# Tyler-Linchenwei/Graph-Distillation-for-Recommendation

Measured on AMD Instinct MI355X. Metric: distill wallclock (SpMM+k-means) & test-acc parity, ogbn-arxiv r=0.5% @1-8 GPU, higher is better.
Workload: dtype fp32

## Files before the change

### graph-distillation-for-recommendation_amd/csrc/gdd_propagate.hip

```cpp
#include <algorithm>
#include <cstdio>
#include <cstdlib>

#include "gdd_common.hpp"

namespace gdd {
namespace {

constexpr int kSeg = GDD_PROP_SEG;
constexpr int kUnroll = 8;

struct Item {
  int32_t row, begin, end, pslot;
};

template <int V>
struct VecT;
template <>
struct VecT<4> {
  using T = float4;
};
template <>
struct VecT<2> {
  using T = float2;
// ... 2 lines not shown
struct VecT<1> {
  using T = float;
};

template <int V>
__device__ __forceinline__ void vload(const float* p, float (&r)[V]) {
  if constexpr (V == 4) {
    float4 t = *reinterpret_cast<const float4*>(p);
    r[0] = t.x; r[1] = t.y; r[2] = t.z; r[3] = t.w;
  } else if constexpr (V == 2) {
    float2 t = *reinterpret_cast<const float2*>(p);
    r[0] = t.x; r[1] = t.y;
  } else {
    r[0] = *p;
  }
}
using f32x4 = __attribute__((ext_vector_type(4))) float;
using f32x2 = __attribute__((ext_vector_type(2))) float;
template <int V>
__device__ __forceinline__ void vload_nt(const float* p, float (&r)[V]) {
  if constexpr (V == 4) {
    f32x4 t = __builtin_nontemporal_load(reinterpret_cast<const f32x4*>(p));
    r[0] = t.x; r[1] = t.y; r[2] = t.z; r[3] = t.w;
  } else if constexpr (V == 2) {
    f32x2 t = __builtin_nontemporal_load(reinterpret_cast<const f32x2*>(p));
    r[0] = t.x; r[1] = t.y;
  } else {
    r[0] = __builtin_nontemporal_load(p);
  }
}
template <int V>
__device__ __forceinline__ void vstore_nt(float* p, const float (&r)[V]) {
  if constexpr (V == 4) {
    f32x4 t = {r[0], r[1], r[2], r[3]};
    __builtin_nontemporal_store(t, reinterpret_cast<f32x4*>(p));
  } else if constexpr (V == 2) {
    f32x2 t = {r[0], r[1]};
    __builtin_nontemporal_store(t, reinterpret_cast<f32x2*>(p));
  } else {
    __builtin_nontemporal_store(r[0], p);
  }
}
template <int V>
__device__ __forceinline__ void vstore(float* p, const float (&r)[V]) {
  if constexpr (V == 4) {
    *reinterpret_cast<float4*>(p) = make_float4(r[0], r[1], r[2], r[3]);
  } else if constexpr (V == 2) {
    *reinterpret_cast<float2*>(p) = make_float2(r[0], r[1]);
  } else {
    *p = r[0];
  }
}

__global__ void k_seg_counts(int64_t n, const int32_t* __restrict__ rowptr,
                             const int32_t* __restrict__ order, const int32_t* __restrict__ rowwise,
                             int32_t* nseg, int32_t* npart) {
  int64_t i = (int64_t)blockIdx.x * blockDim.x + threadIdx.x;
  if (i >= n) return;
  const int64_t r = (order && !(rowwise && *rowwise)) ? order[i] : i;
  int32_t len = rowptr[r + 1] - rowptr[r];
  int32_t s = len <= kSeg ? 1 : (len + kSeg - 1) / kSeg;
  nseg[i] = s;
  npart[i] = s > 1 ? s : 0;
}

__global__ void k_make_items(int64_t n, const int32_t* __restrict__ rowptr,
                             const int32_t* __restrict__ order, const int32_t* __restrict__ rowwise,
                             const int32_t* __restrict__ nseg, const int32_t* __restrict__ item_off,
                             const int32_t* __restrict__ part_off, Item* items,
                             int32_t* long_rows, int32_t* long_off, int32_t* counts) {
  int64_t i = (int64_t)blockIdx.x * blockDim.x + threadIdx.x;
  if (i >= n) return;
  const int32_t r = (order && !(rowwise && *rowwise)) ? order[i] : (int32_t)i;
  const int32_t b = rowptr[r], e = rowptr[r + 1], s = nseg[i], o = item_off[i];
  if (s == 1) {
    items[o] = Item{r, b, e, -1};
  } else {
    const int32_t po = part_off[i];
    for (int32_t k = 0; k < s; ++k) {
      int32_t lo = b + k * kSeg, hi = min(e, lo + kSeg);
      items[o + k] = Item{r, lo, hi, po + k};
    }
    int32_t q = atomicAdd(&counts[1], 1);
    long_rows[q] = r;
    long_off[q] = po;
  }
  if (i == n - 1) counts[0] = o + s;
}

constexpr int kProbeRows = 4096;
constexpr int kProbeCap = 64;
constexpr int kProbeWindow = 4096;
constexpr int64_t kProbeMinRows = 1000000;
__global__ __launch_bounds__(1024) void k_locality_probe(int64_t n, const int32_t* __restrict__ rowptr,
                                                         const int32_t* __restrict__ col,
                                                         int32_t* __restrict__ flag) {
  __shared__ unsigned long long tot[2];
  if (threadIdx.x < 2) tot[threadIdx.x] = 0;
  __syncthreads();
  unsigned near = 0, all = 0;
  const int64_t stride = n / kProbeRows;
  for (int q = threadIdx.x; q < kProbeRows; q += blockDim.x) {
    const int64_t r = q * stride;
    const int32_t b = rowptr[r], e = min(rowptr[r + 1], b + kProbeCap);
    for (int32_t p = b; p < e; ++p) {
      const int64_t dlt = (int64_t)col[p] - r;
      near += (dlt <= kProbeWindow && dlt >= -kProbeWindow) ? 1u : 0u;
    }
    all += (unsigned)(e - b);
  }
  atomicAdd(&tot[0], (unsigned long long)near);
  atomicAdd(&tot[1], (unsigned long long)all);
  __syncthreads();
  if (threadIdx.x == 0) flag[0] = (tot[1] > 0 && 2 * tot[0] >= tot[1]) ? 1 : 0;
}

constexpr int kLenKeyBits = 10;
constexpr int32_t kLenKeyMax = (1 << kLenKeyBits) - 1;
__global__ void k_len_keys(int64_t n, const int32_t* __restrict__ rowptr, int32_t* keys,
                           int32_t* rows) {
  int64_t i = (int64_t)blockIdx.x * blockDim.x + threadIdx.x;
  if (i >= n) return;
  keys[i] = kLenKeyMax - min(rowptr[i + 1] - rowptr[i], kLenKeyMax);
  rows[i] = (int32_t)i;
}

template <int V, int G, int S>
__global__ __launch_bounds__(256) void k_hop(const Item* __restrict__ items,
                                             const int32_t* __restrict__ counts,
                                             const int32_t* __restrict__ col,
                                             const float* __restrict__ val, float scale, int d,
                                             const float* __restrict__ x, float* __restrict__ y,
                                             float* __restrict__ acc_out, float acc_scale,
                                             const float* __restrict__ acc_init,
                                             const float* __restrict__ acc_prev,
                                             float* __restrict__ partials,
                                             const int32_t* __restrict__ ymap,
                                             const int32_t* __restrict__ pmap, int contig) {
  const int lane = threadIdx.x & (G - 1);
  int64_t ib;
  int chunk;
  if constexpr (S > 0) {
    const int xcd = blockIdx.x & 7;
    chunk = xcd % S;
    ib = contig ? (int64_t)xcd * (gridDim.x >> 3) + (blockIdx.x >> 3)
                : (int64_t)(blockIdx.x >> 3) * (8 / S) + xcd / S;
  } else {
    chunk = blockIdx.y;
    ib = blockIdx.x;
  }
  const int64_t g = (ib * blockDim.x + threadIdx.x) / G;
  if (g >= counts[0]) return;
  const Item it = items[g];
  const int f = (chunk * G + lane) * V;
  const bool fa = f < d;
  float acc[V];
#pragma unroll
  for (int v = 0; v < V; ++v) acc[v] = 0.f;

  for (int32_t c0 = it.begin; c0 < it.end; c0 += G) {
    const int32_t p = c0 + lane;
    const bool in = p < it.end;
    const int32_t cj = in ? __builtin_nontemporal_load(col + p) : 0;
    const float vj = in ? scale * __builtin_nontemporal_load(val + p) : 0.f;
    const int cnt = min(G, it.end - c0);
    for (int t = 0; t < cnt; t += kUnroll) {
      float xv[kUnroll][V];
      float vv[kUnroll];
#pragma unroll
      for (int u = 0; u < kUnroll; ++u) {
        const int src = t + u;
        const int32_t jj = __shfl(cj, src < G ? src : 0, G);
        vv[u] = __shfl(vj, src < G ? src : 0, G);
        if (src < cnt && fa) {
          vload<V>(x + (int64_t)jj * d + f, xv[u]);
        } else {
#pragma unroll
          for (int v = 0; v < V; ++v) xv[u][v] = 0.f;
        }
      }
#pragma unroll
      for (int u = 0; u < kUnroll; ++u) {
        if (t + u < cnt) {
#pragma unroll
          for (int v = 0; v < V; ++v) acc[v] = __builtin_fmaf(vv[u], xv[u][v], acc[v]);
        }
      }
    }
  }
  if (!fa) return;
  if (it.pslot < 0) {
    const int64_t o = (int64_t)it.row * d + f;
    const int64_t oy = ymap ? (int64_t)ymap[it.row] * d + f : o;
    vstore<V>(y + oy, acc);
    if (acc_out) {
      float t[V];
      if (acc_init) {
        vload_nt<V>(acc_init + o, t);
#pragma unroll
        for (int v = 0; v < V; ++v) t[v] = acc_scale * t[v];
      } else {
        vload_nt<V>(acc_out + o, t);
      }
      if (acc_prev) {
        float q[V];
        vload<V>(acc_prev + (pmap ? (int64_t)pmap[it.row] * d + f : o), q);
#pragma unroll
        for (int v = 0; v < V; ++v) t[v] = t[v] + acc_scale * q[v];
      }
#pragma unroll
      for (int v = 0; v < V; ++v) t[v] = t[v] + acc_scale * acc[v];
      vstore_nt<V>(acc_out + o, t);
    }
  } else {
    vstore<V>(partials + (int64_t)it.pslot * d + f, acc);
  }
}

constexpr int kFixupBlocks = 1024;
__global__ void k_fixup(const int32_t* __restrict__ counts, const int32_t* __restrict__ long_rows,
                        const int32_t* __restrict__ long_off, const int32_t* __restrict__ rowptr,
                        int d, const float* __restrict__ partials, float* __restrict__ y,
                        float* __restrict__ acc_out, float acc_scale,
                        const float* __restrict__ acc_init, const float* __restrict__ acc_prev,
                        const int32_t* __restrict__ ymap, const int32_t* __restrict__ pmap) {
  const int nl = counts[1];
  for (int r = blockIdx.x; r < nl; r += gridDim.x) {
    const int32_t row = long_rows[r], po = long_off[r];
    const int32_t len = rowptr[row + 1] - rowptr[row];
    const int32_t s = (len + kSeg - 1) / kSeg;
    for (int f = threadIdx.x; f < d; f += blockDim.x) {
      const float* pp = partials + (int64_t)po * d + f;
      float sum = pp[0];
      int32_t k = 1;
      for (; k + 8 <= s; k += 8) {
        float v[8];
#pragma unroll
        for (int u = 0; u < 8; ++u) v[u] = pp[(int64_t)(k + u) * d];
#pragma unroll
        for (int u = 0; u < 8; ++u) sum = sum + v[u];
      }
      for (; k < s; ++k) sum = sum + pp[(int64_t)k * d];
      const int64_t o = (int64_t)row * d + f;
      y[ymap ? (int64_t)ymap[row] * d + f : o] = sum;
      if (acc_out) {
        float t = acc_init ? acc_scale * acc_init[o] : acc_out[o];
        if (acc_prev) t = t + acc_scale * acc_prev[pmap ? (int64_t)pmap[row] * d + f : o];
        acc_out[o] = t + acc_scale * sum;
      }
    }
  }
}

__global__ void k_scale_copy(int64_t total, const float* __restrict__ x, float w,
                             float* __restrict__ target, float* __restrict__ copy) {
  int64_t i = (int64_t)blockIdx.x * blockDim.x + threadIdx.x;
  int64_t stride = (int64_t)gridDim.x * blockDim.x;
  for (; i < total; i += stride) {
    float v = x[i];
    target[i] = w * v;
    if (copy) copy[i] = v;
  }
}

struct Plan {
  Item* items;
  int32_t* counts;
  int32_t* long_rows;
  int32_t* long_off;
  float* partials;
  int64_t max_items;
  int64_t max_long;
  void* sort_ws;
  size_t sort_bytes;
};


inline int64_t max_items_for(int64_t n, int64_t nnz) { return n + nnz / kSeg + 1; }
inline int64_t max_parts_for(int64_t nnz) { return 2 * (nnz / kSeg) + 2; }

constexpr int kLenKeys = kLenKeyMax + 1;
size_t sched_ws_bytes(int64_t n) {
  return align256(sizeof(int32_t) * (kLenKeys + 1)) + align256(gdd_group_ws_bytes(n, kLenKeys));
}

size_t plan_ws_bytes(int64_t n, int64_t nnz, int d) {
  size_t b = 0;
  b += align256(sizeof(int32_t) * n) * 7;
  b += sched_ws_bytes(n);
  b += align256(sizeof(Item) * max_items_for(n, nnz));
  b += align256(sizeof(int32_t) * 4);
  b += align256(sizeof(int32_t) * (nnz / kSeg + 1)) * 2;
  b += align256(sizeof(float) * max_parts_for(nnz) * (size_t)d);
  b += scan_i32_ws_bytes(n) + 256;
  return b + 4096;
}

int carve_plan(int64_t n, int64_t nnz, int d, Carver& cv, Plan& pl, int32_t** tmp, void** scan_ws,
               size_t* scan_bytes) {
  for (int q = 0; q < 7; ++q) tmp[q] = cv.take<int32_t>(n);
  pl.max_items = max_items_for(n, nnz);
  pl.max_long = nnz / kSeg + 1;
  pl.items = cv.take<Item>(pl.max_items);
  pl.counts = cv.take<int32_t>(4);
  pl.long_rows = cv.take<int32_t>(pl.max_long);
  pl.long_off = cv.take<int32_t>(pl.max_long);
  pl.partials = cv.take<float>(max_parts_for(nnz) * (size_t)d);
  *scan_bytes = scan_i32_ws_bytes(n);
  *scan_ws = cv.take<char>(*scan_bytes);
  pl.sort_bytes = sched_ws_bytes(n);
  pl.sort_ws = cv.take<char>(pl.sort_bytes);
  if (!cv.ok()) return fail(GDD_E_WORKSPACE, "propagate: workspace too small");
  return GDD_OK;
}

int build_plan(int64_t n, int64_t nnz, int d, const int32_t* rowptr, const int32_t* col_for_probe,
               Carver& cv, Plan& pl, hipStream_t s, const int32_t* given_order = nullptr) {
  int32_t* tmp[7];
  void* scan_ws;
  size_t sb;
  int rc0 = carve_plan(n, nnz, d, cv, pl, tmp, &scan_ws, &sb);
  if (rc0) return rc0;
  int32_t *nseg = tmp[0], *npart = tmp[1], *item_off = tmp[2], *part_off = tmp[3];
  const unsigned gb = (unsigned)((n + 255) / 256);
  GDD_HIP(hipMemsetAsync(pl.counts, 0, sizeof(int32_t) * 4, s));
  const int32_t* order = given_order;
  const int32_t* rowwise = nullptr;
  if (!given_order && col_for_probe && n >= kProbeMinRows && !forced("hop_no_probe") &&
      !forced("hop_row_order")) {
    k_locality_probe<<<1, 1024, 0, s>>>(n, rowptr, col_for_probe, pl.counts + 2);
    GDD_LAUNCHED();
    rowwise = pl.counts + 2;
  }
  if (!given_order && !forced("hop_row_order")) {
    k_len_keys<<<gb, 256, 0, s>>>(n, rowptr, tmp[4], tmp[5]);
    GDD_LAUNCHED();
    Carver sc(pl.sort_ws, pl.sort_bytes);
    int32_t* key_off = sc.take<int32_t>(kLenKeys + 1);
    const size_t gws = gdd_group_ws_bytes(n, kLenKeys);
    void* gw = sc.take<char>(gws);
    if (!sc.ok()) return fail(GDD_E_WORKSPACE, "propagate: schedule workspace too small");
    int rc = gdd_group_by_label(n, tmp[4], kLenKeys, tmp[6], key_off, gw, gws,
                                reinterpret_cast<gdd_stream_t>(s));
    if (rc) return rc;
    order = tmp[6];
  }
  k_seg_counts<<<gb, 256, 0, s>>>(n, rowptr, order, rowwise, nseg, npart);
  GDD_LAUNCHED();
  int rc = exclusive_scan_i32(nseg, item_off, n, scan_ws, sb, s);
  if (rc) return rc;
  rc = exclusive_scan_i32(npart, part_off, n, scan_ws, sb, s);
  if (rc) return rc;
  k_make_items<<<gb, 256, 0, s>>>(n, rowptr, order, rowwise, nseg, item_off, part_off, pl.items,
                                  pl.long_rows, pl.long_off, pl.counts);
  GDD_LAUNCHED();
  return GDD_OK;
}

struct RowMaps {
  const int32_t* y;
  const int32_t* prev;
};

struct HopForm {
  int V, G, S;
};

HopForm hop_form(int d, int align) {
  if (d <= 0 || (align != 16 && align != 8 && align != 4)) return HopForm{0, 0, 0};
  const int V = (d % 4 == 0 && align == 16) ? 4 : (d % 2 == 0 && align >= 8) ? 2 : 1;
  const int lanes = (d + V - 1) / V;
  const int G = (lanes <= 16 || (V == 4 && lanes > 28 && lanes <= 32)) ? 16 : lanes <= 32 ? 32 : 64;
  const int chunks = (d + G * V - 1) / (G * V);
  const int S = (chunks == 8 || chunks == 4 || chunks == 2 || chunks == 1) ? chunks : 0;
  return HopForm{V, G, S};
}

template <int V, int G, int S>
void launch_hop(const Plan& pl, const int32_t* col, const float* val, float scale, int d,
                const float* x, float* y, float* acc, float acc_scale, const float* acc_init,
                const float* acc_prev, RowMaps rm, hipStream_t s) {
  constexpr int kGroups = 256 / G;
  const int64_t iblocks = (pl.max_items + kGroups - 1) / kGroups;
  if constexpr (S > 0) {
    const int64_t groups = (iblocks + (8 / S) - 1) / (8 / S);
    k_hop<V, G, S><<<(unsigned)(groups * 8), 256, 0, s>>>(pl.items, pl.counts, col, val, scale, d,
                                                          x, y, acc, acc_scale, acc_init, acc_prev,
                                                          pl.partials, rm.y, rm.prev,
                                                          S == 1 && forced("hop_xcd_contig") ? 1 : 0);
  } else {
    const int chunks = (d + G * V - 1) / (G * V);
    k_hop<V, G, 0><<<dim3((unsigned)iblocks, (unsigned)chunks), 256, 0, s>>>(
        pl.items, pl.counts, col, val, scale, d, x, y, acc, acc_scale, acc_init, acc_prev, pl.partials,
        rm.y, rm.prev, 0);
  }
}

template <int V, int G, class... A>
void launch_hop_vg(int S, const A&... a) {
  switch (S) {
    case 8: return launch_hop<V, G, 8>(a...);
    case 4: return launch_hop<V, G, 4>(a...);
    case 2: return launch_hop<V, G, 2>(a...);
    case 1: return launch_hop<V, G, 1>(a...);
    default: return launch_hop<V, G, 0>(a...);
  }
}

template <int V, class... A>
void launch_hop_v(HopForm f, const A&... a) {
  switch (f.G) {
    case 16: return launch_hop_vg<V, 16>(f.S, a...);
    case 32: return launch_hop_vg<V, 32>(f.S, a...);
    default: return launch_hop_vg<V, 64>(f.S, a...);
  }
}

int run_hop(const Plan& pl, const int32_t* rowptr, const int32_t* col, const float* val,
            float scale, int d, const float* x, float* y, float* acc, float acc_scale,
            hipStream_t s, const float* acc_init = nullptr, const float* acc_prev = nullptr,
            RowMaps rm = RowMaps{nullptr, nullptr}) {
  auto aligned = [](const void* p, int a) { return ((uintptr_t)p % a) == 0; };
  const bool a16 = aligned(x, 16) && aligned(y, 16) && (!acc || aligned(acc, 16)) &&
                   (!acc_init || aligned(acc_init, 16)) && (!acc_prev || aligned(acc_prev, 16)) &&
                   aligned(pl.partials, 16);
  const bool a8 = aligned(x, 8) && aligned(y, 8) && (!acc || aligned(acc, 8)) &&
                  (!acc_init || aligned(acc_init, 8)) && (!acc_prev || aligned(acc_prev, 8));
  const HopForm f = hop_form(d, a16 ? 16 : a8 ? 8 : 4);
  switch (f.V) {
    case 4:
      launch_hop_v<4>(f, pl, col, val, scale, d, x, y, acc, acc_scale, acc_init, acc_prev, rm, s);
      break;
    case 2:
      launch_hop_v<2>(f, pl, col, val, scale, d, x, y, acc, acc_scale, acc_init, acc_prev, rm, s);
      break;
    default:
      launch_hop_v<1>(f, pl, col, val, scale, d, x, y, acc, acc_scale, acc_init, acc_prev, rm, s);
      break;
  }
  GDD_LAUNCHED();
  const unsigned fixup_grid = (unsigned)std::min<int64_t>(pl.max_long, kFixupBlocks);
  k_fixup<<<fixup_grid, 256, 0, s>>>(pl.counts, pl.long_rows, pl.long_off, rowptr, d, pl.partials, y,
                                     acc, acc_scale, acc_init, acc_prev, rm.y, rm.prev);
  GDD_LAUNCHED();
  return GDD_OK;
}

int check_csr_args(int64_t n, int64_t nnz, const int32_t* rowptr, const int32_t* col,
                   const float* val, int d) {
  GDD_REQUIRE(n > 0 && n < INT32_MAX, "propagate: n=%lld out of range", (long long)n);
  GDD_REQUIRE(nnz >= 0 && nnz < INT32_MAX, "propagate: nnz=%lld out of range", (long long)nnz);
  GDD_REQUIRE(d > 0, "propagate: d=%d must be positive", d);
  GDD_REQUIRE(rowptr && (nnz == 0 || (col && val)), "propagate: null CSR pointer");
  return GDD_OK;
}

}
}

using namespace gdd;

extern "C" const char* gdd_hop_path(int d, int align) {
  static thread_local char name[32];
  const HopForm f = hop_form(d, align);
  if (f.V == 0) return "invalid";
  snprintf(name, sizeof name, "v%d/g%d/s%d", f.V, f.G, f.S);
  return name;
}

extern "C" size_t gdd_propagate_ws_bytes(int64_t n, int64_t nnz, int d) {
  return plan_ws_bytes(n, nnz, d);
}

extern "C" int gdd_spmm(int64_t n, int64_t nnz, const int32_t* rowptr, const int32_t* col,
                        const float* val, int d, float scale, const float* x, float* y, float* acc,
                        float acc_scale, void* ws, size_t ws_bytes, gdd_stream_t stream) {
  int rc = check_csr_args(n, nnz, rowptr, col, val, d);
  if (rc) return rc;
  GDD_REQUIRE(x && y && ws, "spmm: null pointer");
  hipStream_t s = to_hip(stream);
  Carver cv(ws, ws_bytes);
  Plan pl;
  rc = build_plan(n, nnz, d, rowptr, col, cv, pl, s);
  if (rc) return rc;
  return run_hop(pl, rowptr, col, val, scale, d, x, y, acc, acc_scale, s);
}

extern "C" int gdd_spmm_plan(int64_t n, int64_t nnz, const int32_t* rowptr, int d, void* ws,
                             size_t ws_bytes, gdd_stream_t stream) {
  GDD_REQUIRE(n > 0 && n < INT32_MAX && nnz >= 0 && nnz < INT32_MAX && d > 0 && rowptr && ws,
              "spmm_plan: bad arguments");
  Carver cv(ws, ws_bytes);
  Plan pl;
  return build_plan(n, nnz, d, rowptr, nullptr, cv, pl, to_hip(stream));
}

// ... 120 lines not shown
```

### graph-distillation-for-recommendation_amd/csrc/gdd_kmeanspp.hip

```cpp
#include <algorithm>
#include <climits>
#include <cmath>
#include <cstdlib>

#include <cstring>

#include "gdd_common.hpp"

namespace gdd {
GDD_STAMP_TABLE(kpp)
namespace {

constexpr int kMaxTrials = 16;
constexpr int kBlk = 4096;
constexpr int kThr = 1024;
constexpr int kWaves = kThr / 64;
constexpr int kPer = kBlk / kThr;
constexpr int kBlasThreads = 8;

struct KppState {
  float pot;
  int pad;
};

// ... 1285 lines not shown
      rl[t] = 0.0;
      exl[t] = 0.0;
      if (t < T) {
        float xs[kPer];
#pragma unroll
        for (int q = 0; q < kPer; ++q) xs[q] = s_d[t * kBlk + kPer * tid + q];
        double run = 0.0, r[kPer];
#pragma unroll
        for (int q = 0; q < kPer; ++q) {
          const int64_t e = j0 + kPer * tid + q;
          run = run + (e < n ? (double)(wv(a.w, e) * xs[q]) : 0.0);
          r[q] = run;
        }
        double inc = run;
#pragma unroll
        for (int o = 1; o < 64; o <<= 1) {
          const double y = __shfl_up(inc, o);
          if (lane >= o) inc = inc + y;
        }
        double ex = __shfl_up(inc, 1);
        if (lane == 0) ex = 0.0;
        if (lane == 63) s_wt[t][wave] = inc;
        exl[t] = ex;
#pragma unroll
        for (int q = 0; q < kPer; ++q)
          if (q == (int)(last % kPer)) rl[t] = r[q];
      }
    }
    __syncthreads();
    if (owner) {
#pragma unroll
      for (int t = 0; t < kSplitMaxT; ++t) {
        if (t < T) {
          double B = 0.0;
          for (int q = 0; q < wave; ++q) B = B + s_wt[t][q];
          a.fsum[cq][(int64_t)t * a.nblk + blk] = (B + exl[t]) + rl[t];
        }
      }
    }
  }
  GDD_STAMP_WHEN(g_stamps_kpp, (tid == 0 && c == 5 && (blk == 0 || blk == a.nblk - 1)), blk == 0 ? 34 : 44);
  const int64_t NB = min<int64_t>(kBlk, a.m1 - j0);
  if (NB > 0 && wave < T) {
    const float v = sgemv_block_wave(s_d + wave * kBlk, a.w ? a.w + j0 : nullptr, NB, wave, T);
    if (lane == 0) a.vblk[cq][(int64_t)wave * a.nblk + blk] = v;
  }
  GDD_STAMP_WHEN(g_stamps_kpp, (lane == 0 && wave == 0 && c == 5 && (blk == 0 || blk == a.nblk - 1)),
                 blk == 0 ? 35 : 45);
#ifdef GDD_STAMPS
  if (lane == 0 && c == 5) atomicMax(&g_stamps_kpp[46], (unsigned long long)__builtin_amdgcn_s_memrealtime());
#endif
}

__global__ __launch_bounds__(kThr) void k_kpp_final(KppArgs a, int c) {
  __shared__ float s_pot[kMaxTrials];
  const int q = c & 1;
  const int b = fold_round(a, q, s_pot);
  const int64_t src = a.cand[q][b];
  if (threadIdx.x == 0) a.indices[c] = src;
  for (int j = threadIdx.x; j < a.dim; j += kThr) a.centers[(int64_t)c * a.dim + j] = a.X[src * a.dim + j];
}

constexpr int kTg = 2;
constexpr int kPts = 64;

struct Kpp1Args {
  int64_t n, m1;
  int dim, T, k, pad;
  const float* X;
  const float* XT;
  const float* w;
  const double* xsq;
  const float* closest0;
  const KppState* st;
  const double* uniforms;
  float* dist[2];
  float* potv[2];
  int64_t* candw[2];
  int64_t* candself[2];
  int64_t* candr[2];
  double* candn[2];
  int* win;
  unsigned* counter;
  float* centers;
  int64_t* indices;
  SklPlan plan;
  float* dist2[2];
  float* potv2[2];
  int64_t* candw2[2];
  int64_t* candself2[2];
  int exact;
};

__device__ __forceinline__ int kpp1_argmin(const float* __restrict__ pot, int T) {
  int b = 0;
  for (int q = 1; q < T; ++q) {
    const float pb = pot[b], pt = pot[q];
    if (pb == pb && (pt < pb || pt != pt)) b = q;
  }
  return b;
}

template <bool SEQ>
__global__ __launch_bounds__(256) void k_kpp1_dist(Kpp1Args a, int c) {
  extern __shared__ double s_cr[];
  __shared__ int64_t s_cw[kMaxTrials * kMaxTrials];
// ... 1641 lines not shown
  const SklPlan p{n, B, T, dim, 0, 0};
  const int64_t ms[2] = {std::min(n, B), n > B ? n % B : 0};
  for (int64_t m : ms)
    if (m > 0 && !skl_chunk_seq(p, m)) return false;
  return true;
}

}
}

using namespace gdd;

extern "C" int gdd_skl_sqdist(int n_rows, const float* C, int64_t n, int dim, const float* X,
                              float* out, gdd_stream_t stream) {
  GDD_REQUIRE(n_rows >= 1 && n > 0 && dim > 0 && dim <= 4096, "skl_sqdist: invalid shape");
  GDD_REQUIRE(n <= (int64_t)INT_MAX * kThr, "skl_sqdist: n too large");
  GDD_REQUIRE(C && X && out, "skl_sqdist: null pointer");
  SklPlan p{n, skl_batch_size(n_rows, n, dim), n_rows, dim, 0, 0};
  p.all_seq = skl_all_seq(n, n_rows, dim, p.B) ? 1 : 0;
  const size_t lds = sizeof(double) * (size_t)dim;
  k_skl_sqdist<<<dim3((unsigned)((n + kThr - 1) / kThr), (unsigned)n_rows), kThr, lds,
                 to_hip(stream)>>>(p, C, X, out);
  GDD_LAUNCHED();
  return GDD_OK;
}

namespace {

enum KppPath {
  KPP_FIRST_ONLY,
  KPP_SINGLE_TABLE_PAIR,
  KPP_SINGLE_TABLE,
  KPP_SINGLE_FUSED,
  KPP_SINGLE_TWO_LAUNCH,
  KPP_SPLIT,
  KPP_BIG_PAIR,
  KPP_BIG,
  KPP_BLOCK_TABLE,
  KPP_BLOCK,
};

struct KppPlan {
  int64_t n, nblk;
  int dim, T, k;
  KppPath path;
  bool seq;
  int64_t B, B1;
  int exact;
  int overlap;
  int ept;
  size_t lds;
  size_t lds1;
  size_t lds_split;
  size_t lds_big;
  bool xt;
  bool xt_before_init;
  bool xt_after_first;
  bool Dbig;
  bool Dm;
  bool pairs;
};

constexpr int64_t kDmBigMax = 32768;
constexpr int64_t kBig1Default = 16384;
bool kpp_table_pays(int64_t n, int dim, int k) {
  return (double)(k - 1) * 2.5e7 >= (double)n * (double)n * (double)dim;
}

KppPlan kpp_plan(int64_t n, int dim_in, int n_trials, int k_in) {
  KppPlan p{};
  const int dim = p.dim = std::max(dim_in, 1);
  const int T = p.T = std::max(n_trials, 1);
  const int k = p.k = std::max(k_in, 1);
  p.n = n;
  p.nblk = (n + kBlk - 1) / kBlk;
  p.B = skl_batch_size(T, n, dim);
  p.B1 = skl_batch_size(1, n, dim);
  p.seq = skl_all_seq(n, T, dim, p.B);
  const char* ex = getenv("GDD_KPP_EXACT");
  p.exact = ex ? atoi(ex) : 1;
  p.overlap = forced("kpp_pair_serial") ? 0 : 1;
  p.ept = n <= (int64_t)kBigThr * 8 ? 8 : n <= (int64_t)kBigThr * 16 ? 16 : 32;
  p.lds = sizeof(double) * (size_t)dim + sizeof(float) * (kBlk + kChainPad);
  p.lds1 = sizeof(double) * (size_t)T * std::max(dim, 48);
  p.lds_split = sizeof(double) * (size_t)T * dim + sizeof(float) * (size_t)T * kBlk;
  p.lds_big = sizeof(float) * ((size_t)kBigThr * p.ept + kChainPad);

  const bool no_table = forced("kpp_no_table"), single_round = forced("kpp_single_round");
  const bool table_shape = dim <= kDmX && T >= 2 && k >= kDmMinK;
  p.xt = n <= kBlk || n * (int64_t)dim < INT_MAX;
  p.Dm = n <= kBlk && table_shape;
  p.Dbig = n > kBlk && n <= kDmBigMax && table_shape && !no_table &&
           (kpp_table_pays(n, dim, k) || forced("kpp_force_table")) && p.seq;
  p.pairs = p.Dm || (p.Dbig && T <= kPairMaxT && n <= (int64_t)kBigThr * 8);

  const bool single = p.nblk == 1 && T >= 2;
  p.xt_before_init = p.xt && n > kBlk;
  p.xt_after_first = single && p.seq && k > 1;
  const int64_t big1_max = std::min((int64_t)forced_value("kpp_big1_max", (double)kBig1Default), kBig1Max);
  const bool big1 = n <= big1_max && T >= 2 && !forced("kpp_no_big1");
  const bool split = p.seq && p.xt_before_init && T >= 2 && T <= kSplitMaxT && p.lds_split <= 150 * 1024 &&
                     p.nblk >= kSplitMinBlocks && !forced("kpp_no_split");
  if (k == 1) {
    p.path = KPP_FIRST_ONLY;
  } else if (single) {
    const int64_t fused_grid = (n + kFPts - 1) / kFPts * T;
    if (p.seq && p.Dm && !no_table)
      p.path = T <= kPairMaxT && !single_round ? KPP_SINGLE_TABLE_PAIR : KPP_SINGLE_TABLE;
    else if (dim <= kMaxDimF && fused_grid <= 256 && !forced("kpp_two_launch"))
      p.path = KPP_SINGLE_FUSED;
    else
      p.path = KPP_SINGLE_TWO_LAUNCH;
  } else if (split) {
    p.path = KPP_SPLIT;
  } else if (p.Dbig && p.xt_before_init) {
    p.path = !big1 ? KPP_BLOCK_TABLE : p.pairs && !single_round ? KPP_BIG_PAIR : KPP_BIG;
  } else {
    p.path = KPP_BLOCK;
  }
  return p;
}

const char* kpp_path_name(const KppPlan& p) {
  switch (p.path) {
    case KPP_FIRST_ONLY: return "first_only";
    case KPP_SINGLE_TABLE_PAIR: return "single_table_pair";
    case KPP_SINGLE_TABLE: return "single_table";
    case KPP_SINGLE_FUSED: return p.seq ? "single_fused/seq" : "single_fused/blas";
    case KPP_SINGLE_TWO_LAUNCH: return p.seq ? "single_two_launch/seq" : "single_two_launch/blas";
    case KPP_SPLIT: return "split";
    case KPP_BIG_PAIR: return "big_pair";
    case KPP_BIG: return "big";
    case KPP_BLOCK_TABLE: return "block_table";
    case KPP_BLOCK: return p.seq ? "block/seq" : "block/blas";
  }
  return "invalid";
}

struct KppBufs {
  KppState* st;
  double* xsq;
  float* closest0;
  double* fsum0;
  float* XT;
  float* Dbig;
  float* Dm;
};

void kpp_carve(const KppPlan& p, Carver& cv, KppBufs* bf, KppArgs* a, Kpp1Args* b1) {
  const size_t n = (size_t)p.n, nblk = (size_t)p.nblk, T = (size_t)p.T;
  bf->st = cv.take<KppState>(1);
  bf->xsq = cv.take<double>(n);
  bf->closest0 = cv.take<float>(n);
  bf->fsum0 = cv.take<double>(nblk);
  for (int q = 0; q < 2; ++q) a->dist[q] = cv.take<float>(n * T);
// ... 144 lines not shown
  struct {
    Kpp1Args b1;
    const float* Dm;
    int k, overlap;
  } key;
  std::memset(&key, 0, sizeof(key));
  key.b1 = b1;
  key.Dm = Dm;
  key.k = p.k;
  key.overlap = overlap;
  return replay_or_run("kpp_pair_chain", &key, sizeof(key), s, chain);
}

int kpp_single_table(const KppPlan& p, const KppBufs& bf, const Kpp1Args& b1, hipStream_t s) {
  if (const int rc = launch_kpp_dmat(p.n, p.dim, b1.X, bf.XT, bf.xsq, bf.Dm, s)) return rc;
  for (int c = 1; c < p.k; ++c) {
    k_kpp1_dm<<<(unsigned)p.T, 256, 0, s>>>(b1, bf.Dm, c);
    GDD_LAUNCHED();
  }
  return kpp1_finish(b1, s);
}

int kpp_single_fused(const KppPlan& p, const Kpp1Args& b1, hipStream_t s) {
  const dim3 gf((unsigned)((p.n + kFPts - 1) / kFPts), (unsigned)p.T);
  GDD_HIP(hipMemsetAsync(b1.counter, 0, sizeof(unsigned) * (size_t)p.k * p.T, s));
  for (int c = 1; c < p.k; ++c) {
    if (p.seq)
      k_kpp1_fused<true><<<gf, 256, 0, s>>>(b1, c);
    else
      k_kpp1_fused<false><<<gf, 256, 0, s>>>(b1, c);
    GDD_LAUNCHED();
  }
  return kpp1_finish(b1, s);
}

int kpp_single_two_launch(const KppPlan& p, const Kpp1Args& b1, hipStream_t s) {
  const dim3 g1((unsigned)((p.n + kPts - 1) / kPts), (unsigned)(((p.T + kTg - 1) / kTg + 3) / 4));
  for (int c = 1; c < p.k; ++c) {
    if (p.seq)
      k_kpp1_dist<true><<<g1, 256, p.lds1, s>>>(b1, c);
    else
      k_kpp1_dist<false><<<g1, 256, p.lds1, s>>>(b1, c);
    GDD_LAUNCHED();
    k_kpp1_pick<<<p.T, kThr, 0, s>>>(b1, c);
    GDD_LAUNCHED();
  }
  k_kpp1_final<<<1, 64, 0, s>>>(b1, p.k - 1);
  GDD_LAUNCHED();
  return GDD_OK;
}

int kpp_split(const KppPlan& p, const KppArgs& a, hipStream_t s) {
  void (*dists)(KppArgs, int) = nullptr;
  switch (p.T) {
    case 2: dists = k_kpp_dists<2>; break;
    case 3: dists = k_kpp_dists<3>; break;
    case 4: dists = k_kpp_dists<4>; break;
    case 5: dists = k_kpp_dists<5>; break;
    case 6: dists = k_kpp_dists<6>; break;
    case 7: dists = k_kpp_dists<7>; break;
    default: dists = k_kpp_dists<8>; break;
  }
  if (const int rc = kpp_max_lds((const void*)dists, p.lds_split)) return rc;
  for (int c = 1; c < p.k; ++c) {
    k_kpp_round<true, true><<<dim3(1, p.T), kThr, p.lds, s>>>(a, c);
    GDD_LAUNCHED();
    dists<<<(unsigned)p.nblk, kThr, p.lds_split, s>>>(a, c);
    GDD_LAUNCHED();
  }
  return kpp_finish(p, a, s);
}

typedef void (*KppBigFn)(Kpp1Args, const float*, int);
int kpp_big_begin(const KppPlan& p, const KppArgs& a, const KppBufs& bf, Kpp1Args& b1, KppBigFn* big,
                  hipStream_t s) {
  if (const int rc = launch_kpp_dmat(p.n, p.dim, a.X, bf.XT, bf.xsq, bf.Dbig, s)) return rc;
  kpp1_fill(b1, p, a, nullptr);
  KppBigFn f = k_kpp1_big<8>;
  if (p.ept == 16) f = k_kpp1_big<16>;
  if (p.ept == 32) f = k_kpp1_big<32>;
  if (const int rc = kpp_max_lds((const void*)f, p.lds_big)) return rc;
  f<<<1, kBigThr, p.lds_big, s>>>(b1, bf.Dbig, 0);
  GDD_LAUNCHED();
  *big = f;
  return GDD_OK;
}

int kpp_big_pair(const KppPlan& p, const KppArgs& a, const KppBufs& bf, Kpp1Args& b1, hipStream_t s) {
  KppBigFn big;
  if (const int rc = kpp_big_begin(p, a, bf, b1, &big, s)) return rc;
  void (*big2)(Kpp1Args, const float*, int, int, int) = k_kpp1_big2<8>;
  if (const int rc = kpp_max_lds((const void*)big2, p.lds_big)) return rc;
  return kpp1_pair_rounds(b1, s, [&](unsigned grid, int c, int lq, int pair) {
    big2<<<grid, kBigThr, p.lds_big, s>>>(b1, bf.Dbig, c, lq, pair);
  });
}

int kpp_big(const KppPlan& p, const KppArgs& a, const KppBufs& bf, Kpp1Args& b1, hipStream_t s) {
  KppBigFn big;
  if (const int rc = kpp_big_begin(p, a, bf, b1, &big, s)) return rc;
  for (int c = 1; c < p.k; ++c) {
    big<<<(unsigned)p.T, kBigThr, p.lds_big, s>>>(b1, bf.Dbig, c);
    GDD_LAUNCHED();
  }
  return kpp1_finish(b1, s);
}

int kpp_block(const KppPlan& p, const KppArgs& a, hipStream_t s) {
  for (int c = 1; c < p.k; ++c) {
    if (p.seq)
      k_kpp_round<true><<<dim3((unsigned)p.nblk, p.T), kThr, p.lds, s>>>(a, c);
    else
      k_kpp_round<false><<<dim3((unsigned)p.nblk, p.T), kThr, p.lds, s>>>(a, c);
    GDD_LAUNCHED();
    if (p.T == 1) {
      k_kpp_pot1<<<1, 64, 0, s>>>(p.n, a.dist[c & 1], a.w, a.pot1 + (c & 1));
      GDD_LAUNCHED();
    }
  }
  return kpp_finish(p, a, s);
}
// ... 87 lines not shown
```

Before: 14.65 million.

## Fold long-row partials in-kernel via last-arriver counters, drop fixup kernel

Long rows split into segments no longer go through a separate fixup kernel. Each segment writes its partial with a write-through store and bumps a per-row, per-chunk atomic counter. The last segment to arrive sums all partials and writes y and the accumulator epilogue directly, then resets the counter. This removes one kernel launch and the long-row list built with atomics, at the cost of a wait on stores plus an atomic per segment, and it depends on memory-ordering assumptions (inline asm store with sc1, agent-scope fences) being correct.

```diff
diff --git a/graph-distillation-for-recommendation_amd/csrc/gdd_propagate.hip b/graph-distillation-for-recommendation_amd/csrc/gdd_propagate.hip
--- a/graph-distillation-for-recommendation_amd/csrc/gdd_propagate.hip
+++ b/graph-distillation-for-recommendation_amd/csrc/gdd_propagate.hip
@@ -78,6 +78,21 @@
   }
 }
 
+template <int V>
+__device__ __forceinline__ void vstore_wt(float* p, const float (&r)[V]) {
+  if constexpr (V == 4) {
+    f32x4 t = {r[0], r[1], r[2], r[3]};
+    asm volatile("global_store_dwordx4 %0, %1, off sc1\n\ts_nop 1" ::"v"(p), "v"(t) : "memory");
+  } else if constexpr (V == 2) {
+    const unsigned long long t =
+        ((unsigned long long)__float_as_uint(r[1]) << 32) | (unsigned long long)__float_as_uint(r[0]);
+    __hip_atomic_store(reinterpret_cast<unsigned long long*>(p), t, __ATOMIC_RELAXED,
+                       __HIP_MEMORY_SCOPE_AGENT);
+  } else {
+    __hip_atomic_store(p, r[0], __ATOMIC_RELAXED, __HIP_MEMORY_SCOPE_AGENT);
+  }
+}
+
 __global__ void k_seg_counts(int64_t n, const int32_t* __restrict__ rowptr,
                              const int32_t* __restrict__ order, const int32_t* __restrict__ rowwise,
                              int32_t* nseg, int32_t* npart) {
@@ -94,7 +109,7 @@
                              const int32_t* __restrict__ order, const int32_t* __restrict__ rowwise,
                              const int32_t* __restrict__ nseg, const int32_t* __restrict__ item_off,
                              const int32_t* __restrict__ part_off, Item* items,
-                             int32_t* long_rows, int32_t* long_off, int32_t* counts) {
+                             int32_t* fold_ctr, int ctr_stride, int32_t* counts) {
   int64_t i = (int64_t)blockIdx.x * blockDim.x + threadIdx.x;
   if (i >= n) return;
   const int32_t r = (order && !(rowwise && *rowwise)) ? order[i] : (int32_t)i;
@@ -107,9 +122,7 @@
       int32_t lo = b + k * kSeg, hi = min(e, lo + kSeg);
       items[o + k] = Item{r, lo, hi, po + k};
     }
-    int32_t q = atomicAdd(&counts[1], 1);
-    long_rows[q] = r;
-    long_off[q] = po;
+    for (int c = 0; c < ctr_stride; ++c) fold_ctr[(int64_t)po * ctr_stride + c] = 0;
   }
   if (i == n - 1) counts[0] = o + s;
 }
@@ -154,6 +167,7 @@
 template <int V, int G, int S>
 __global__ __launch_bounds__(256) void k_hop(const Item* __restrict__ items,
                                              const int32_t* __restrict__ counts,
+                                             const int32_t* __restrict__ rowptr,
                                              const int32_t* __restrict__ col,
                                              const float* __restrict__ val, float scale, int d,
                                              const float* __restrict__ x, float* __restrict__ y,
@@ -161,6 +175,7 @@
                                              const float* __restrict__ acc_init,
                                              const float* __restrict__ acc_prev,
                                              float* __restrict__ partials,
+                                             int32_t* __restrict__ fold_ctr, int ctr_stride,
                                              const int32_t* __restrict__ ymap,
                                              const int32_t* __restrict__ pmap, int contig) {
   const int lane = threadIdx.x & (G - 1);
@@ -215,66 +230,69 @@
     }
   }
   if (!fa) return;
-  if (it.pslot < 0) {
-    const int64_t o = (int64_t)it.row * d + f;
-    const int64_t oy = ymap ? (int64_t)ymap[it.row] * d + f : o;
-    vstore<V>(y + oy, acc);
-    if (acc_out) {
-      float t[V];
-      if (acc_init) {
-        vload_nt<V>(acc_init + o, t);
-#pragma unroll
-        for (int v = 0; v < V; ++v) t[v] = acc_scale * t[v];
-      } else {
-        vload_nt<V>(acc_out + o, t);
+  if (it.pslot >= 0) {
+    const int32_t rb = rowptr[it.row];
+    const int32_t nseg = (rowptr[it.row + 1] - rb + kSeg - 1) / kSeg;
+    const int32_t po = it.pslot - (it.begin - rb) / kSeg;
+    float* mine = partials + (int64_t)it.pslot * d + f;
+    vstore_wt<V>(mine, acc);
+    asm volatile("s_waitcnt vmcnt(0)" ::: "memory");
+    int32_t* ctr = fold_ctr + (int64_t)po * ctr_stride + chunk;
+    int32_t arrived = 0;
+    if (lane == 0)
+      arrived = __hip_atomic_fetch_add(ctr, 1, __ATOMIC_RELAXED, __HIP_MEMORY_SCOPE_AGENT);
+    arrived = __shfl(arrived, 0, G);
+    if (arrived != nseg - 1) return;
+    __builtin_amdgcn_fence(__ATOMIC_ACQUIRE, "agent");
+    const float* pp = partials + (int64_t)po * d + f;
+#pragma unroll
+    for (int v = 0; v < V; ++v)
+      acc[v] = __hip_atomic_load(pp + v, __ATOMIC_RELAXED, __HIP_MEMORY_SCOPE_AGENT);
+    int32_t k = 1;
+    for (; k + 8 <= nseg; k += 8) {
+      float pv[8][V];
+#pragma unroll
+      for (int u = 0; u < 8; ++u) {
+#pragma unroll
+        for (int v = 0; v < V; ++v)
+          pv[u][v] = __hip_atomic_load(pp + (int64_t)(k + u) * d + v, __ATOMIC_RELAXED,
+                                       __HIP_MEMORY_SCOPE_AGENT);
       }
-      if (acc_prev) {
-        float q[V];
-        vload<V>(acc_prev + (pmap ? (int64_t)pmap[it.row] * d + f : o), q);
-#pragma unroll
-        for (int v = 0; v < V; ++v) t[v] = t[v] + acc_scale * q[v];
+#pragma unroll
+      for (int u = 0; u < 8; ++u) {
+#pragma unroll
+        for (int v = 0; v < V; ++v) acc[v] = acc[v] + pv[u][v];
       }
-#pragma unroll
-      for (int v = 0; v < V; ++v) t[v] = t[v] + acc_scale * acc[v];
-      vstore_nt<V>(acc_out + o, t);
-    }
-  } else {
-    vstore<V>(partials + (int64_t)it.pslot * d + f, acc);
-  }
-}
-
-constexpr int kFixupBlocks = 1024;
-__global__ void k_fixup(const int32_t* __restrict__ counts, const int32_t* __restrict__ long_rows,
-                        const int32_t* __restrict__ long_off, const int32_t* __restrict__ rowptr,
-                        int d, const float* __restrict__ partials, float* __restrict__ y,
-                        float* __restrict__ acc_out, float acc_scale,
-                        const float* __restrict__ acc_init, const float* __restrict__ acc_prev,
-                        const int32_t* __restrict__ ymap, const int32_t* __restrict__ pmap) {
-  const int nl = counts[1];
-  for (int r = blockIdx.x; r < nl; r += gridDim.x) {
-    const int32_t row = long_rows[r], po = long_off[r];
-    const int32_t len = rowptr[row + 1] - rowptr[row];
-    const int32_t s = (len + kSeg - 1) / kSeg;
-    for (int f = threadIdx.x; f < d; f += blockDim.x) {
-      const float* pp = partials + (int64_t)po * d + f;
-      float sum = pp[0];
-      int32_t k = 1;
-      for (; k + 8 <= s; k += 8) {
-        float v[8];
-#pragma unroll
-        for (int u = 0; u < 8; ++u) v[u] = pp[(int64_t)(k + u) * d];
-#pragma unroll
-        for (int u = 0; u < 8; ++u) sum = sum + v[u];
-      }
-      for (; k < s; ++k) sum = sum + pp[(int64_t)k * d];
-      const int64_t o = (int64_t)row * d + f;
-      y[ymap ? (int64_t)ymap[row] * d + f : o] = sum;
-      if (acc_out) {
-        float t = acc_init ? acc_scale * acc_init[o] : acc_out[o];
-        if (acc_prev) t = t + acc_scale * acc_prev[pmap ? (int64_t)pmap[row] * d + f : o];
-        acc_out[o] = t + acc_scale * sum;
-      }
-    }
+    }
+    for (; k < nseg; ++k) {
+#pragma unroll
+      for (int v = 0; v < V; ++v)
+        acc[v] = acc[v] + __hip_atomic_load(pp + (int64_t)k * d + v, __ATOMIC_RELAXED,
+                                            __HIP_MEMORY_SCOPE_AGENT);
+    }
+    if (lane == 0) __hip_atomic_store(ctr, 0, __ATOMIC_RELAXED, __HIP_MEMORY_SCOPE_AGENT);
+  }
+  const int64_t o = (int64_t)it.row * d + f;
+  const int64_t oy = ymap ? (int64_t)ymap[it.row] * d + f : o;
+  vstore<V>(y + oy, acc);
+  if (acc_out) {
+    float t[V];
+    if (acc_init) {
+      vload_nt<V>(acc_init + o, t);
+#pragma unroll
+      for (int v = 0; v < V; ++v) t[v] = acc_scale * t[v];
+    } else {
+      vload_nt<V>(acc_out + o, t);
+    }
+    if (acc_prev) {
+      float q[V];
+      vload<V>(acc_prev + (pmap ? (int64_t)pmap[it.row] * d + f : o), q);
+#pragma unroll
+      for (int v = 0; v < V; ++v) t[v] = t[v] + acc_scale * q[v];
+    }
+#pragma unroll
+    for (int v = 0; v < V; ++v) t[v] = t[v] + acc_scale * acc[v];
+    vstore_nt<V>(acc_out + o, t);
   }
 }
 
@@ -292,11 +310,10 @@
 struct Plan {
   Item* items;
   int32_t* counts;
-  int32_t* long_rows;
-  int32_t* long_off;
   float* partials;
+  int32_t* fold_ctr;
+  int ctr_stride;
   int64_t max_items;
-  int64_t max_long;
   void* sort_ws;
   size_t sort_bytes;
 };
@@ -304,6 +321,7 @@
 
 inline int64_t max_items_for(int64_t n, int64_t nnz) { return n + nnz / kSeg + 1; }
 inline int64_t max_parts_for(int64_t nnz) { return 2 * (nnz / kSeg) + 2; }
+inline int ctr_stride_for(int d) { return std::max(2, (d + 63) / 64); }
 
 constexpr int kLenKeys = kLenKeyMax + 1;
 size_t sched_ws_bytes(int64_t n) {
@@ -316,7 +334,7 @@
   b += sched_ws_bytes(n);
   b += align256(sizeof(Item) * max_items_for(n, nnz));
   b += align256(sizeof(int32_t) * 4);
-  b += align256(sizeof(int32_t) * (nnz / kSeg + 1)) * 2;
+  b += align256(sizeof(int32_t) * max_parts_for(nnz) * (size_t)ctr_stride_for(d));
   b += align256(sizeof(float) * max_parts_for(nnz) * (size_t)d);
   b += scan_i32_ws_bytes(n) + 256;
   return b + 4096;
@@ -326,12 +344,11 @@
                size_t* scan_bytes) {
   for (int q = 0; q < 7; ++q) tmp[q] = cv.take<int32_t>(n);
   pl.max_items = max_items_for(n, nnz);
-  pl.max_long = nnz / kSeg + 1;
   pl.items = cv.take<Item>(pl.max_items);
   pl.counts = cv.take<int32_t>(4);
-  pl.long_rows = cv.take<int32_t>(pl.max_long);
-  pl.long_off = cv.take<int32_t>(pl.max_long);
   pl.partials = cv.take<float>(max_parts_for(nnz) * (size_t)d);
+  pl.ctr_stride = ctr_stride_for(d);
+  pl.fold_ctr = cv.take<int32_t>(max_parts_for(nnz) * (size_t)pl.ctr_stride);
   *scan_bytes = scan_i32_ws_bytes(n);
   *scan_ws = cv.take<char>(*scan_bytes);
   pl.sort_bytes = sched_ws_bytes(n);
@@ -378,7 +395,7 @@
   rc = exclusive_scan_i32(npart, part_off, n, scan_ws, sb, s);
   if (rc) return rc;
   k_make_items<<<gb, 256, 0, s>>>(n, rowptr, order, rowwise, nseg, item_off, part_off, pl.items,
-                                  pl.long_rows, pl.long_off, pl.counts);
+                                  pl.fold_ctr, pl.ctr_stride, pl.counts);
   GDD_LAUNCHED();
   return GDD_OK;
 }
@@ -403,22 +420,22 @@
 }
 
 template <int V, int G, int S>
-void launch_hop(const Plan& pl, const int32_t* col, const float* val, float scale, int d,
+void launch_hop(const Plan& pl, const int32_t* rowptr, const int32_t* col, const float* val, float scale, int d,
                 const float* x, float* y, float* acc, float acc_scale, const float* acc_init,
                 const float* acc_prev, RowMaps rm, hipStream_t s) {
   constexpr int kGroups = 256 / G;
   const int64_t iblocks = (pl.max_items + kGroups - 1) / kGroups;
   if constexpr (S > 0) {
     const int64_t groups = (iblocks + (8 / S) - 1) / (8 / S);
-    k_hop<V, G, S><<<(unsigned)(groups * 8), 256, 0, s>>>(pl.items, pl.counts, col, val, scale, d,
-                                                          x, y, acc, acc_scale, acc_init, acc_prev,
-                                                          pl.partials, rm.y, rm.prev,
-                                                          S == 1 && forced("hop_xcd_contig") ? 1 : 0);
+    k_hop<V, G, S><<<(unsigned)(groups * 8), 256, 0, s>>>(
+        pl.items, pl.counts, rowptr, col, val, scale, d, x, y, acc, acc_scale, acc_init, acc_prev,
+        pl.partials, pl.fold_ctr, pl.ctr_stride, rm.y, rm.prev,
+        S == 1 && forced("hop_xcd_contig") ? 1 : 0);
   } else {
     const int chunks = (d + G * V - 1) / (G * V);
     k_hop<V, G, 0><<<dim3((unsigned)iblocks, (unsigned)chunks), 256, 0, s>>>(
-        pl.items, pl.counts, col, val, scale, d, x, y, acc, acc_scale, acc_init, acc_prev, pl.partials,
-        rm.y, rm.prev, 0);
+        pl.items, pl.counts, rowptr, col, val, scale, d, x, y, acc, acc_scale, acc_init, acc_prev,
+        pl.partials, pl.fold_ctr, pl.ctr_stride, rm.y, rm.prev, 0);
   }
 }
 
@@ -455,19 +472,15 @@
   const HopForm f = hop_form(d, a16 ? 16 : a8 ? 8 : 4);
   switch (f.V) {
     case 4:
-      launch_hop_v<4>(f, pl, col, val, scale, d, x, y, acc, acc_scale, acc_init, acc_prev, rm, s);
+      launch_hop_v<4>(f, pl, rowptr, col, val, scale, d, x, y, acc, acc_scale, acc_init, acc_prev, rm, s);
       break;
     case 2:
-      launch_hop_v<2>(f, pl, col, val, scale, d, x, y, acc, acc_scale, acc_init, acc_prev, rm, s);
+      launch_hop_v<2>(f, pl, rowptr, col, val, scale, d, x, y, acc, acc_scale, acc_init, acc_prev, rm, s);
       break;
     default:
-      launch_hop_v<1>(f, pl, col, val, scale, d, x, y, acc, acc_scale, acc_init, acc_prev, rm, s);
+      launch_hop_v<1>(f, pl, rowptr, col, val, scale, d, x, y, acc, acc_scale, acc_init, acc_prev, rm, s);
       break;
   }
-  GDD_LAUNCHED();
-  const unsigned fixup_grid = (unsigned)std::min<int64_t>(pl.max_long, kFixupBlocks);
-  k_fixup<<<fixup_grid, 256, 0, s>>>(pl.counts, pl.long_rows, pl.long_off, rowptr, d, pl.partials, y,
-                                     acc, acc_scale, acc_init, acc_prev, rm.y, rm.prev);
   GDD_LAUNCHED();
   return GDD_OK;
 }
```

Result: slower. 14.46 million (-1.3%).

## Split fused k-means++ distance kernel into row-distance and block-terms kernels

Applied to the files above, without the earlier changes.

The split k-means++ path previously ran one fused kernel per block computing candidate distances, prefix sums and sgemv terms. By default it now launches two kernels per round. The first is a smaller 256-thread row kernel that computes the clamped min-distances with a register prefetch over dimensions. The second is a block-terms kernel gridded over blocks and trial groups that does the prefix and sgemv reductions. This aims at better occupancy and parallelism, and the fused kernel stays available behind a flag. In exchange it adds an extra launch per round and a round-trip of the distance rows through global memory.

```diff
diff --git a/graph-distillation-for-recommendation_amd/csrc/gdd_kmeanspp.hip b/graph-distillation-for-recommendation_amd/csrc/gdd_kmeanspp.hip
--- a/graph-distillation-for-recommendation_amd/csrc/gdd_kmeanspp.hip
+++ b/graph-distillation-for-recommendation_amd/csrc/gdd_kmeanspp.hip
@@ -1361,6 +1361,161 @@
 #endif
 }
 
+constexpr int kRowsThr = 256;
+constexpr int kRowsPts = kRowsThr * kPer;
+template <int T>
+__global__ __launch_bounds__(kRowsThr) void k_kpp_dist_rows(KppArgs a, int c) {
+  extern __shared__ double s_cs[];
+  __shared__ double s_cn[kSplitMaxT];
+  const int tile = blockIdx.x, tid = threadIdx.x;
+  const int dim = a.dim;
+  const int pq = (c - 1) & 1, cq = c & 1;
+  const int64_t n = a.n, j0 = (int64_t)tile * kRowsPts;
+  const float* wrow = c == 1 ? a.closest0 : a.dist[pq] + (int64_t)a.winq[cq] * n;
+  const bool stamp = tid == 0 && c == 5 && (tile == 0 || tile == (int)gridDim.x - 1);
+  (void)stamp;
+  GDD_STAMP_WHEN(g_stamps_kpp, stamp, tile == 0 ? 30 : 40);
+  const float* __restrict__ xt = a.XT + j0;
+  uint32_t off[kPer];
+  double dot[kSplitMaxT][kPer];
+#pragma unroll
+  for (int q = 0; q < kPer; ++q) {
+    const int64_t i = j0 + tid + kRowsThr * q;
+    off[q] = i < n ? (uint32_t)(tid + kRowsThr * q) : 0u;
+#pragma unroll
+    for (int t = 0; t < kSplitMaxT; ++t) dot[t][q] = 0.0;
+  }
+  constexpr int D = 3;
+  float buf[D][kPer];
+#pragma unroll
+  for (int d = 0; d < D; ++d)
+    if (d < dim) {
+#pragma unroll
+      for (int q = 0; q < kPer; ++q) buf[d][q] = (xt + (int64_t)d * n)[off[q]];
+    }
+  float wv_[kPer];
+  double xs[kPer];
+#pragma unroll
+  for (int q = 0; q < kPer; ++q) {
+    wv_[q] = wrow[j0 + off[q]];
+    xs[q] = a.xsq[j0 + off[q]];
+  }
+  for (int e = tid; e < T * dim; e += kRowsThr) {
+    const int t = e / dim, j = e - t * dim;
+    s_cs[e] = (double)a.X[a.cand[cq][t] * dim + j];
+  }
+  if (tid < T) s_cn[tid] = a.xsq[a.cand[cq][tid]];
+  __syncthreads();
+  GDD_STAMP_WHEN(g_stamps_kpp, stamp, tile == 0 ? 31 : 41);
+  for (int j0f = 0; j0f < dim; j0f += D) {
+#pragma unroll
+    for (int d = 0; d < D; ++d) {
+      const int j = j0f + d;
+      if (j >= dim) break;
+      float u[kPer];
+#pragma unroll
+      for (int q = 0; q < kPer; ++q) u[q] = buf[d][q];
+      if (j + D < dim) {
+#pragma unroll
+        for (int q = 0; q < kPer; ++q) buf[d][q] = (xt + (int64_t)(j + D) * n)[off[q]];
+      }
+#pragma unroll
+      for (int t = 0; t < kSplitMaxT; ++t)
+        if (t < T) {
+          const double cv = s_cs[t * dim + j];
+#pragma unroll
+          for (int q = 0; q < kPer; ++q) dot[t][q] = __builtin_fma(cv, (double)u[q], dot[t][q]);
+        }
+    }
+  }
+  GDD_STAMP_WHEN(g_stamps_kpp, stamp, tile == 0 ? 32 : 42);
+#pragma unroll
+  for (int t = 0; t < kSplitMaxT; ++t) {
+    if (t >= T) break;
+    float* drow = a.dist[cq] + (int64_t)t * n;
+#pragma unroll
+    for (int q = 0; q < kPer; ++q) {
+      const int64_t i = j0 + tid + kRowsThr * q;
+      if (i < n) {
+        float f = (float)(((-2.0 * dot[t][q]) + s_cn[t]) + xs[q]);
+        f = f < 0.f ? 0.f : f;
+        drow[i] = np_minimum(wv_[q], f);
+      }
+    }
+  }
+  GDD_STAMP_WHEN(g_stamps_kpp, stamp, tile == 0 ? 33 : 43);
+#ifdef GDD_STAMPS
+  if ((tid & 63) == 0 && c == 5) atomicMax(&g_stamps_kpp[46], (unsigned long long)__builtin_amdgcn_s_memrealtime());
+#endif
+}
+
+constexpr int kTermsTrials = 2;
+__global__ __launch_bounds__(kThr) void k_kpp_block_terms(KppArgs a, int c, int tw) {
+  extern __shared__ float s_rows[];
+  __shared__ double s_wave[kWaves];
+  const int blk = blockIdx.x, t0 = blockIdx.y * tw, tid = threadIdx.x, wave = tid >> 6, lane = tid & 63;
+  const int cq = c & 1;
+  const int nt = min(tw, a.T - t0);
+  const int64_t n = a.n, j0 = (int64_t)blk * kBlk;
+  const bool stamp = c == 5 && (blk == 0 || blk == a.nblk - 1) && t0 == 0;
+  (void)stamp;
+  GDD_STAMP_WHEN(g_stamps_kpp, (stamp && tid == 0), blk == 0 ? 50 : 55);
+  float x[kTermsTrials][kPer];
+  float w4[kPer];
+#pragma unroll
+  for (int q = 0; q < kPer; ++q) {
+    const int64_t e = j0 + kPer * tid + q;
+    w4[q] = e < n ? wv(a.w, e) : 0.f;
+  }
+#pragma unroll
+  for (int r = 0; r < kTermsTrials; ++r) {
+    const float* row = a.dist[cq] + (int64_t)(t0 + r) * n;
+#pragma unroll
+    for (int q = 0; q < kPer; ++q) {
+      const int64_t e = j0 + kPer * tid + q;
+      x[r][q] = r < nt && e < n ? row[e] : 0.f;
+    }
+  }
+#pragma unroll
+  for (int r = 0; r < kTermsTrials; ++r)
+    if (r < nt) {
+#pragma unroll
+      for (int q = 0; q < kPer; ++q) s_rows[r * kBlk + kPer * tid + q] = x[r][q];
+    }
+  __syncthreads();
+  GDD_STAMP_WHEN(g_stamps_kpp, (stamp && tid == 0), blk == 0 ? 51 : 56);
+  const int64_t last = min<int64_t>(n, j0 + kBlk) - 1 - j0;
+  const bool owner = tid == (int)(last / kPer);
+#pragma unroll
+  for (int r = 0; r < kTermsTrials; ++r) {
+    if (r >= nt) break;
+    double v[kPer], pre[kPer];
+#pragma unroll
+    for (int q = 0; q < kPer; ++q) {
+      const int64_t e = j0 + kPer * tid + q;
+      v[q] = e < n ? (double)(w4[q] * x[r][q]) : 0.0;
+    }
+    block_prefix(v, pre, s_wave);
+    if (owner) {
+      double tot = 0.0;
+#pragma unroll
+      for (int q = 0; q < kPer; ++q)
+        if (q == (int)(last % kPer)) tot = pre[q];
+      a.fsum[cq][(int64_t)(t0 + r) * a.nblk + blk] = tot;
+    }
+  }
+  GDD_STAMP_WHEN(g_stamps_kpp, (stamp && tid == 0), blk == 0 ? 52 : 57);
+  const int64_t NB = min<int64_t>(kBlk, a.m1 - j0);
+  if (NB > 0 && wave < nt) {
+    const float y = sgemv_block_wave(s_rows + wave * kBlk, a.w ? a.w + j0 : nullptr, NB, t0 + wave, a.T);
+    if (lane == 0) a.vblk[cq][(int64_t)(t0 + wave) * a.nblk + blk] = y;
+  }
+  GDD_STAMP_WHEN(g_stamps_kpp, (stamp && tid == 0), blk == 0 ? 53 : 58);
+#ifdef GDD_STAMPS
+  if (lane == 0 && c == 5) atomicMax(&g_stamps_kpp[47], (unsigned long long)__builtin_amdgcn_s_memrealtime());
+#endif
+}
+
 __global__ __launch_bounds__(kThr) void k_kpp_final(KppArgs a, int c) {
   __shared__ float s_pot[kMaxTrials];
   const int q = c & 1;
@@ -3108,6 +3263,7 @@
   size_t lds;
   size_t lds1;
   size_t lds_split;
+  bool split_fused;
   size_t lds_big;
   bool xt;
   bool xt_before_init;
@@ -3155,8 +3311,11 @@
   p.xt_after_first = single && p.seq && k > 1;
   const int64_t big1_max = std::min((int64_t)forced_value("kpp_big1_max", (double)kBig1Default), kBig1Max);
   const bool big1 = n <= big1_max && T >= 2 && !forced("kpp_no_big1");
+  const double smb = forced_value("kpp_split_min_blocks", (double)kSplitMinBlocks);
+  const int64_t split_min_blocks = smb >= 1.0 && smb < 9e15 ? (int64_t)smb : kSplitMinBlocks;
   const bool split = p.seq && p.xt_before_init && T >= 2 && T <= kSplitMaxT && p.lds_split <= 150 * 1024 &&
-                     p.nblk >= kSplitMinBlocks && !forced("kpp_no_split");
+                     p.nblk >= split_min_blocks && !forced("kpp_no_split");
+  p.split_fused = forced("kpp_split_fused");
   if (k == 1) {
     p.path = KPP_FIRST_ONLY;
   } else if (single) {
@@ -3407,21 +3566,42 @@
 
 int kpp_split(const KppPlan& p, const KppArgs& a, hipStream_t s) {
   void (*dists)(KppArgs, int) = nullptr;
+  void (*rows)(KppArgs, int) = nullptr;
   switch (p.T) {
-    case 2: dists = k_kpp_dists<2>; break;
-    case 3: dists = k_kpp_dists<3>; break;
-    case 4: dists = k_kpp_dists<4>; break;
-    case 5: dists = k_kpp_dists<5>; break;
-    case 6: dists = k_kpp_dists<6>; break;
-    case 7: dists = k_kpp_dists<7>; break;
-    default: dists = k_kpp_dists<8>; break;
-  }
-  if (const int rc = kpp_max_lds((const void*)dists, p.lds_split)) return rc;
+#define GDD_KPP_SPLIT_T(t)      \
+  dists = k_kpp_dists<t>;       \
+  rows = k_kpp_dist_rows<t>;    \
+  break
+    case 2: GDD_KPP_SPLIT_T(2);
+    case 3: GDD_KPP_SPLIT_T(3);
+    case 4: GDD_KPP_SPLIT_T(4);
+    case 5: GDD_KPP_SPLIT_T(5);
+    case 6: GDD_KPP_SPLIT_T(6);
+    case 7: GDD_KPP_SPLIT_T(7);
+    default: GDD_KPP_SPLIT_T(8);
+#undef GDD_KPP_SPLIT_T
+  }
+  const int tgroups = (p.T + kTermsTrials - 1) / kTermsTrials, tw = (p.T + tgroups - 1) / tgroups;
+  const size_t lds_rows = sizeof(double) * (size_t)p.T * p.dim, lds_terms = sizeof(float) * (size_t)tw * kBlk;
+  if (p.split_fused) {
+    if (const int rc = kpp_max_lds((const void*)dists, p.lds_split)) return rc;
+  } else {
+    if (const int rc = kpp_max_lds((const void*)rows, lds_rows)) return rc;
+    if (const int rc = kpp_max_lds((const void*)k_kpp_block_terms, lds_terms)) return rc;
+  }
+  const unsigned ntile = (unsigned)((p.n + kRowsPts - 1) / kRowsPts);
   for (int c = 1; c < p.k; ++c) {
     k_kpp_round<true, true><<<dim3(1, p.T), kThr, p.lds, s>>>(a, c);
     GDD_LAUNCHED();
-    dists<<<(unsigned)p.nblk, kThr, p.lds_split, s>>>(a, c);
-    GDD_LAUNCHED();
+    if (p.split_fused) {
+      dists<<<(unsigned)p.nblk, kThr, p.lds_split, s>>>(a, c);
+      GDD_LAUNCHED();
+    } else {
+      rows<<<ntile, kRowsThr, lds_rows, s>>>(a, c);
+      GDD_LAUNCHED();
+      k_kpp_block_terms<<<dim3((unsigned)p.nblk, tgroups), kThr, lds_terms, s>>>(a, c, tw);
+      GDD_LAUNCHED();
+    }
   }
   return kpp_finish(p, a, s);
 }
```

Result: no change. 14.51 million before, 14.57 million after, median of 3 (+0.4%).
